# willi-menapace/PlayableEnvironments

Hardware: AMD Instinct MI355X
Metric: Mrays/s (higher is better)
Workload: dtype f32; 1 GPU; tennis renderer, 256x256 frame per GPU (rank r renders the frame of seed 1234 + r), 4 objects, 64+128 hierarchical samples/ray (coarse+fine networks), eval - BASELINE.json configs[1]; rays_per_gpu=65536, frames_per_gpu=1, parallelism=frame shard x1

## Files before the change

playableenvironments_amd/csrc/mlp.hip:

```cpp
#include "pr_common.h"
#include "mlp_tile.h"

#include <cstddef>

#include <stdarg.h>
#include <stdlib.h>

namespace pr {


int compute_dims(const pr_object_model_t& m, ModelDims* d) {
    PR_REQUIRE(m.kind == 0 || m.kind == 1, "unknown nerf model kind %d", m.kind);
    PR_REQUIRE(m.octaves >= 0 && m.octaves <= PR_MAX_OCTAVES, "octaves %d out of range", m.octaves);
    d->din = m.kind == 0 ? 3 : 6;
    d->enc = d->din + 2 * d->din * m.octaves;
    d->enc_pad = round_up(d->enc, 32);
    d->W = m.layers_width;
    d->Wpad = round_up(d->W, 32);
    d->W2 = m.layers_width / 2;
    d->W2pad = round_up(d->W2, 32);
    d->F = m.output_features;
    d->Fpad = round_up(d->F, 32);
    PR_REQUIRE(d->enc_pad <= MAX_ENC, "encoding width %d exceeds %d", d->enc, MAX_ENC);
    PR_REQUIRE(d->W >= 2 && d->Wpad <= MAX_WIDTH, "layers_width %d unsupported (max %d)", d->W, MAX_WIDTH);
// ... 397 lines not shown
        if (first) {
            row[ch] = g;
            row[p.Wpad + ch] = b;
        } else {
            row[2 * p.Wpad + ch] = g;
            row[2 * p.Wpad + p.W2pad + ch] = b;
        }
    }
}

__global__ __launch_bounds__(256) void k_adain_fold(FoldParams p) { adain_fold_body(p); }

struct FoldGroup { FoldParams job[PR_MAX_OBJECTS]; };
__global__ __launch_bounds__(256) void k_adain_fold_group(FoldGroup g) {
    const FoldParams& p = g.job[blockIdx.z];
    if ((int)blockIdx.x >= p.frames || (int)blockIdx.y * 256 >= p.Wpad + p.W2pad) return;
    adain_fold_body(p);
}

int launch_adain_fold(const FoldParams& p, hipStream_t s) {
    PR_REQUIRE(p.affine1.weight && p.affine1.bias && p.affine4.weight && p.affine4.bias && p.bn1_mean && p.bn1_var &&
                   p.bn4_mean && p.bn4_var,
               "AdaIN parameters missing");
    PR_REQUIRE(p.affine1.out_features == 2 * p.W && p.affine1.in_features == p.S, "features_head.1 affine shape");
    PR_REQUIRE(p.affine4.out_features == 2 * p.W2 && p.affine4.in_features == p.S, "features_head.4 affine shape");
    hipLaunchKernelGGL(k_adain_fold, dim3(p.frames, (p.Wpad + p.W2pad + 255) / 256), dim3(256), 0, s, p);
    PR_LAUNCH_CHECK();
    return PR_OK;
}

int launch_adain_fold_group(const FoldParams* jobs, int count, hipStream_t s) {
    PR_REQUIRE(count >= 1 && count <= PR_MAX_OBJECTS, "adain fold group: %d objects", count);
    static thread_local FoldGroup g;
    int frames = 0, blocks = 0;
    for (int k = 0; k < count; ++k) {
        const FoldParams& p = jobs[k];
        PR_REQUIRE(p.affine1.weight && p.affine1.bias && p.affine4.weight && p.affine4.bias && p.bn1_mean && p.bn1_var &&
                       p.bn4_mean && p.bn4_var,
                   "AdaIN parameters missing");
        PR_REQUIRE(p.affine1.out_features == 2 * p.W && p.affine1.in_features == p.S, "features_head.1 affine shape");
        PR_REQUIRE(p.affine4.out_features == 2 * p.W2 && p.affine4.in_features == p.S, "features_head.4 affine shape");
        g.job[k] = p;
        frames = std::max(frames, p.frames);
        blocks = std::max(blocks, (p.Wpad + p.W2pad + 255) / 256);
    }
    hipLaunchKernelGGL(k_adain_fold_group, dim3(frames, blocks, count), dim3(256), 0, s, g);
    PR_LAUNCH_CHECK();
    return PR_OK;
}


__device__ __forceinline__ void head_on_tile(Smem& S, const MlpParams& p, EncRegs& enc, int valid_rows) {
    for (int l = p.n_backbone; l < p.n_layers; ++l) run_layer(p.layers[l], S, p, 0, 0, enc);
    write_rows_indirect(S, p.feat, p.F, p.F, p.ones_col);
    if (threadIdx.x == 0 && p.head_count) atomicAdd(p.head_count, valid_rows);
    __syncthreads();
}

__device__ __forceinline__ int gated_head(Smem& S, const MlpParams& p, int tile_base, int pending, EncRegs& enc) {
    const int tid = threadIdx.x, lane = tid & 63;
    const unsigned long long live = __ballot((S.flags[lane] & 4) != 0);
    const int L = __popcll(live);
    float* pact = p.pend_act + (size_t)blockIdx.x * TILE_M * p.Wpad;
    int* pmeta = p.pend_meta + (size_t)blockIdx.x * TILE_M * 2;
    const unsigned long long below = (1ull << lane) - 1ull;
    const int w4 = p.Wpad >> 2;
    if (L == 0) {
        __syncthreads();
        return pending;
    }
    if (pending + L >= TILE_M) {
        const int need = TILE_M - L;
        if (tid == 0) S.uniform_frame = 1;
        if (tid < TILE_M) {
            if ((live >> tid) & 1ull) {
                S.dest[tid] = tile_base + tid;
                S.src[tid] = -1;
            } else {
                const int slot = pending - need + __popcll(~live & below);
                S.src[tid] = slot;
                S.dest[tid] = pmeta[2 * slot];
                S.frame[tid] = pmeta[2 * slot + 1];
            }
        }
        __syncthreads();
        if (need) {
            for (int idx = tid; idx < TILE_M * w4; idx += MLP_THREADS) {
                const int row = idx / w4, c = (idx - row * w4) * 4;
                const int slot = S.src[row];
                if (slot >= 0)
                    *reinterpret_cast<float4*>(S.X + row * LDX + c) = *reinterpret_cast<const float4*>(pact + (size_t)slot * p.Wpad + c);
            }
        }
        if (tid < TILE_M && S.frame[tid] != S.frame[0]) S.uniform_frame = 0;
        __syncthreads();
        head_on_tile(S, p, enc, TILE_M);
        return pending - need;
    }
    if (tid < TILE_M) {
        int slot = -1;
        if ((live >> tid) & 1ull) {
            slot = pending + __popcll(live & below);
            pmeta[2 * slot] = tile_base + tid;
            pmeta[2 * slot + 1] = S.frame[tid];
        }
        S.src[tid] = slot;
    }
    __syncthreads();
    for (int idx = tid; idx < TILE_M * w4; idx += MLP_THREADS) {
        const int row = idx / w4, c = (idx - row * w4) * 4;
        const int slot = S.src[row];
        if (slot >= 0)
            *reinterpret_cast<float4*>(pact + (size_t)slot * p.Wpad + c) = *reinterpret_cast<const float4*>(S.X + row * LDX + c);
    }
    __syncthreads();
    return pending + L;
}

__device__ __forceinline__ void gated_head_flush(Smem& S, const MlpParams& p, int pending, EncRegs& enc) {
    if (pending <= 0) return;
    const int tid = threadIdx.x;
    const float* pact = p.pend_act + (size_t)blockIdx.x * TILE_M * p.Wpad;
    const int* pmeta = p.pend_meta + (size_t)blockIdx.x * TILE_M * 2;
    const int w4 = p.Wpad >> 2;
    if (tid == 0) S.uniform_frame = 1;
    if (tid < TILE_M) {
        const bool has = tid < pending;
        S.dest[tid] = has ? pmeta[2 * tid] : -1;
        S.frame[tid] = pmeta[2 * (has ? tid : 0) + 1];
    }
    __syncthreads();
    for (int idx = tid; idx < pending * w4; idx += MLP_THREADS) {
        const int row = idx / w4, c = (idx - row * w4) * 4;
        *reinterpret_cast<float4*>(S.X + row * LDX + c) = *reinterpret_cast<const float4*>(pact + (size_t)row * p.Wpad + c);
    }
    if (tid < TILE_M && S.frame[tid] != S.frame[0]) S.uniform_frame = 0;
    __syncthreads();
    head_on_tile(S, p, enc, pending);
}


__device__ __forceinline__ void count_stat_rows(const Smem& S, const MlpParams& p) {
    if (p.phase == 1 && threadIdx.x < 64) {
        const int alive = __popcll(__ballot((S.flags[threadIdx.x] & 3) == 3));
        if (threadIdx.x == 0 && alive) atomicAdd(p.stat_count, alive);
    }
}

__device__ __forceinline__ void flush_column_stats(const ColumnStats& cs, const MlpParams& p, int nblk) {
    const int wave = threadIdx.x >> 6, lane = threadIdx.x & 63;
    if (lane >= 32) return;
#pragma unroll
    for (int blk = 0; blk < 2; ++blk) {
        const int cb = wave + blk * MLP_WAVES;
        if (cb >= nblk) continue;
        const int col = cb * 32 + lane;
        const double s1 = blk ? cs.s1[1] : cs.s1[0], s2 = blk ? cs.s2[1] : cs.s2[0];
        if (s1 != 0.0 || s2 != 0.0) {
            atomicAdd(p.stats + col, s1);
            atomicAdd(p.stats + p.h_out_width + col, s2);
        }
    }
}

#ifdef PR_MLP_TRACE
__device__ unsigned long long g_mlp_trace[1024][12];
#define PR_TRACE_MARK(i) if (threadIdx.x == 0) g_mlp_trace[blockIdx.x][i] = wall_clock64()
#else
#define PR_TRACE_MARK(i)
#endif

template <bool TRAIN, bool GROUP, bool SPLIT = false, bool SIGMA_ONLY = false>
__device__ __forceinline__ void mlp_tile_loop(const MlpParams& p) {
    extern __shared__ __attribute__((aligned(16))) char smem_raw[];
    Smem& S = *reinterpret_cast<Smem*>(smem_raw);
    const int tid = threadIdx.x;
    const int total = *p.total;
    PR_PHASE_BEGIN();
    if (GROUP) {
        __syncthreads();
        if (tid == 0) S.next_tile = atomicAdd(p.tile_counter, 1);
    }
    for (int i = tid; i <= p.Wpad; i += MLP_THREADS) S.head_w[i] = p.sigma_w[i];
    __syncthreads();
    int pending = 0;
    EncRegs enc;
    ColumnStats cstats;
    cstats.s1[0] = cstats.s1[1] = cstats.s2[0] = cstats.s2[1] = 0.0;
    const bool dynamic_tiles = GROUP || (!TRAIN && p.tile_counter != nullptr);
    for (int tile = GROUP ? S.next_tile : (int)blockIdx.x; tile * TILE_M < total; tile = S.next_tile) {
        const int tile_base = tile * TILE_M;
        PR_PHASE_T0();
#ifdef PR_MLP_TRACE
        if (GROUP && !TRAIN && tid == 0) g_mlp_trace[blockIdx.x][5 + (p.positions == 4 ? 0 : 1)] += 1;
#endif
        int claimed = 0;
        if (tid == 0) S.uniform_frame = 1;
        if (SPLIT && tid == 0) S.tile_max[0] = S.tile_max[1] = 0;
        if (tid < TILE_M) {
            const int idx = tile_base + tid;
            const bool valid = idx < total;
            const int src = valid ? idx : tile_base;
            const int flat = p.rec_flat[src];
            const int frame = flat / p.samples_per_frame;
            S.flat[tid] = flat;
            S.frame[tid] = frame;
            S.flags[tid] = valid ? 3 : 0;
            if (p.kind == 0) {
                S.pos[tid * 8 + 0] = p.rec_pos[(size_t)src * 3 + 0];
                S.pos[tid * 8 + 1] = p.rec_pos[(size_t)src * 3 + 1];
                S.pos[tid * 8 + 2] = p.rec_pos[(size_t)src * 3 + 2];
            } else {
                const int ray = (flat - frame * p.samples_per_frame) / p.positions;
                const ObjRay rr = object_ray(p.w2o + (size_t)frame * p.w2o_stride, p.ray_origins + (size_t)frame * 3,
                                             p.ray_directions + ((size_t)frame * p.rays + ray) * 3);
                const float nrm = sqrtf(__fadd_rn(__fadd_rn(__fmul_rn(rr.d[0], rr.d[0]), __fmul_rn(rr.d[1], rr.d[1])),
                                                  __fmul_rn(rr.d[2], rr.d[2])));
                for (int a = 0; a < 3; ++a) {
                    S.pos[tid * 8 + a] = __fdiv_rn(rr.o[a], p.size[a]);
                    S.pos[tid * 8 + 3 + a] = __fdiv_rn(rr.d[a], nrm);
                }
            }
        }
        __syncthreads();
        if (tid < TILE_M && S.frame[tid] != S.frame[0]) S.uniform_frame = 0;
        PR_PHASE(0);

        int cur = p.has_bender ? 0 : 1;
        if (p.has_bender) {
            fill_bender_input(S, p, enc, false, SPLIT ? &S.tile_max[0] : nullptr);
            __syncthreads();
            if (TRAIN && p.save_bin) write_tile_rows(S, p.save_bin, p.bin_pad, p.bin_pad, tile_base, false);
            for (int l = 0; l < p.b_count; ++l) {
                if (TRAIN) {
                    run_layer<false, true, false, SPLIT>(p.b_layers[l], S, p, tile_base, 1, enc, nullptr,
                                           p.save_bbits ? reinterpret_cast<unsigned long long*>(p.save_bbits + (size_t)l * p.save_bbits_stride) +
                                                              (size_t)tile * p.BWpad : nullptr, nullptr, &cur);
                } else {
                    run_layer(p.b_layers[l], S, p, tile_base, 1, enc);
                }
                if (TRAIN && p.save_bact) write_tile_rows(S, p.save_bact + (size_t)l * p.save_bact_stride, p.BWpad, p.BWpad, tile_base, false);
            }
            if (SPLIT && tid == 0) S.tile_max[cur ^ 1] = 0;
            for (int s = tid >> 3; s < TILE_M; s += MLP_THREADS / 8) {
                float out[3];
                row_dots(S, s, as_global(p.b_out), p.BWpad, p.BWpad, 3, out);
                if ((tid & 7) != 0) continue;
                float d[3], bent[3];
                if (TRAIN && p.save_braw && (S.flags[s] & 1))
                    for (int a = 0; a < 3; ++a) p.save_braw[(size_t)(tile_base + s) * 3 + a] = out[a];
                for (int a = 0; a < 3; ++a) {
                    const float x = S.pos[s * 8 + a];
                    float dl = __fmul_rn(out[a], p.size[a]);
                    dl = nan_max(dl, __fsub_rn(p.lo[a], x));
                    dl = nan_min(dl, __fsub_rn(p.hi[a], x));
                    if (p.canonical) dl = __fmul_rn(dl, 0.0f);
                    d[a] = dl;
                    bent[a] = __fadd_rn(x, dl);
                    S.pos[s * 8 + a] = bent[a];
                }
                if (S.flags[s] & 1) {
                    if (p.dispmag)
                        p.dispmag[S.flat[s]] = sqrtf(__fadd_rn(__fadd_rn(__fmul_rn(d[0], d[0]), __fmul_rn(d[1], d[1])),
                                                               __fmul_rn(d[2], d[2])));
                    if (TRAIN && p.save_delta)
                        for (int a = 0; a < 3; ++a) p.save_delta[(size_t)(tile_base + s) * 3 + a] = d[a];
                    if (p.delta_dense)
                        for (int a = 0; a < 3; ++a) p.delta_dense[(size_t)S.flat[s] * 3 + a] = d[a];
                    if (!in_box(bent[0], bent[1], bent[2], p.lo, p.hi)) S.flags[s] &= ~2;
                }
            }
            __syncthreads();
        }

        PR_PHASE(1);
        fill_nerf_input(S, p, enc, false, SPLIT ? &S.tile_max[cur ^ 1] : nullptr);
        cur ^= 1;
        __syncthreads();
        PR_PHASE(2);
        if (TRAIN && p.save_enc) write_tile_rows(S, p.save_enc, p.enc_pad, p.enc_pad, tile_base, false);

        for (int l = 0; l < p.n_backbone; ++l) {
            if (TRAIN) {
                run_layer<false, true, false, SPLIT>(p.layers[l], S, p, tile_base, 0, enc, nullptr,
                                       p.save_bits
                                           ? reinterpret_cast<unsigned long long*>(p.save_bits + (size_t)l * p.save_bits_stride) + (size_t)tile * p.Wpad
                                           : nullptr, nullptr, &cur);
            } else {
                run_layer(p.layers[l], S, p, tile_base, 0, enc);
            }
            PR_PHASE(10);
            if (TRAIN && p.save_act)
                write_tile_rows(S, p.save_act + (size_t)l * p.save_act_stride, p.Wpad, p.Wpad, tile_base, false);
            PR_PHASE(11);
        }

        PR_PHASE(15);
        if (dynamic_tiles && tid == 0) claimed = atomicAdd(p.tile_counter, 1);
        if (p.kind == 0) {
            for (int s = tid >> 3; s < TILE_M; s += MLP_THREADS / 8) {
                float sg;
                row_dots(S, s, S.head_w, p.Wpad, p.Wpad, 1, &sg);
                if ((tid & 7) == 0 && (S.flags[s] & 3) == 3) {
                    const float sv = p.in_scene[(size_t)S.frame[s] * p.in_scene_stride] ? sg + S.head_w[p.Wpad] : p.empty_alpha;
                    p.sigma[S.flat[s]] = sv;
                    if (!(sv <= 0.f)) S.flags[s] |= 4;
                }
            }
        } else if (tid < TILE_M) {
            if (S.flags[tid] & 1) {
                const bool present = p.in_scene[(size_t)S.frame[tid] * p.in_scene_stride] != 0;
                p.sigma[S.flat[tid]] = present ? 10.0f : p.empty_alpha;
                if (present || !(p.empty_alpha <= 0.f)) S.flags[tid] |= 4;
            }
        }

        if (tid == 0) S.next_tile = GROUP ? claimed : (dynamic_tiles ? (int)gridDim.x + claimed : tile + (int)gridDim.x);
        PR_PHASE(7);
        if (SIGMA_ONLY) {
            __syncthreads();
        } else if (!TRAIN && p.gate) {
            __syncthreads();
            if (!(p.empty_alpha <= 0.f)) {
                for (int idx = tid; idx < TILE_M * p.F; idx += MLP_THREADS) {
                    const int row = idx / p.F;
                    if ((S.flags[row] & 3) == 1) p.feat[(size_t)(tile_base + row) * p.F + (idx - row * p.F)] = 0.f;
                }
            }
            pending = gated_head(S, p, tile_base, pending, enc);
            PR_PHASE(8);
        } else if (!TRAIN) {
            for (int l = p.n_backbone; l < p.n_layers; ++l) run_layer(p.layers[l], S, p, tile_base, 0, enc);
            PR_PHASE(15);
            write_tile_rows(S, p.feat, p.F, p.F, tile_base, true, p.ones_col);
            __syncthreads();
            PR_PHASE(8);
        } else {
            Layer raw = p.layers[p.n_backbone];
            raw.epi = EPI_FEATURES;
            run_layer<false, false, true, SPLIT>(raw, S, p, tile_base, 0, enc, nullptr, nullptr, &cstats, &cur);
            PR_PHASE(12);
            if (tid < TILE_M && (S.flags[tid] & 1)) p.row_flags[tile_base + tid] = S.flags[tid];
            write_tile_rows(S, p.h_out, p.h_out_width, p.h_out_width, tile_base, false);
            count_stat_rows(S, p);
            PR_PHASE(13);
            __syncthreads();
            PR_PHASE(14);
        }
    }
    if (!TRAIN && !SIGMA_ONLY && p.gate) gated_head_flush(S, p, pending, enc);
    if (TRAIN) flush_column_stats(cstats, p, p.layers[p.n_backbone].nblk);
    PR_PHASE_FLUSH();
}

__global__ __launch_bounds__(MLP_THREADS, MLP_BLOCKS_PER_CU) void k_mlp_mfma(MlpParams p) { mlp_tile_loop<false, false>(p); }
__global__ __launch_bounds__(MLP_THREADS, MLP_BLOCKS_PER_CU) void k_mlp_mfma_train(MlpParams p) { mlp_tile_loop<true, false>(p); }
__global__ __launch_bounds__(MLP_THREADS, MLP_BLOCKS_PER_CU) void k_mlp_sigma(MlpParams p) { mlp_tile_loop<false, false, false, true>(p); }
__global__ __launch_bounds__(MLP_THREADS, MLP_BLOCKS_PER_CU) void k_mlp_mfma_group(MlpParams j0, MlpParams j1, MlpParams j2, MlpParams j3,
                                                                                   int count) {
    PR_TRACE_MARK(0);
    mlp_tile_loop<false, true>(j0);
    PR_TRACE_MARK(1);
    if (count > 1) mlp_tile_loop<false, true>(j1);
    PR_TRACE_MARK(2);
    if (count > 2) mlp_tile_loop<false, true>(j2);
    PR_TRACE_MARK(3);
    if (count > 3) mlp_tile_loop<false, true>(j3);
    PR_TRACE_MARK(4);
}

__global__ __launch_bounds__(MLP_THREADS, MLP_BLOCKS_PER_CU) void k_mlp_sigma_group(MlpParams j0, MlpParams j1, MlpParams j2, MlpParams j3,
                                                                                    int count) {
    mlp_tile_loop<false, true, false, true>(j0);
    if (count > 1) mlp_tile_loop<false, true, false, true>(j1);
    if (count > 2) mlp_tile_loop<false, true, false, true>(j2);
    if (count > 3) mlp_tile_loop<false, true, false, true>(j3);
}

#ifdef PR_MLP_TRACE
extern "C" int pr_debug_mlp_trace(unsigned long long* out) {
    (void)hipDeviceSynchronize();
    return hipMemcpyFromSymbol(out, HIP_SYMBOL(g_mlp_trace), sizeof(unsigned long long) * 1024 * 12) == hipSuccess ? 0 : 1;
}
#endif

__global__ __launch_bounds__(MLP_THREADS, MLP_BLOCKS_PER_CU) void k_mlp_mfma_train_group(MlpParams j0, MlpParams j1, MlpParams j2, MlpParams j3,
                                                                                         int count) {
    mlp_tile_loop<true, true>(j0);
    if (count > 1) mlp_tile_loop<true, true>(j1);
// ... 627 lines not shown
    PR_LAUNCH_CHECK();
    return PR_OK;
}

int launch_chain_bwd(const ChainBwdParams& c, int max_rows, hipStream_t s) {
    if (max_rows <= 0) return PR_OK;
    int cu_count = 0;
    PR_TRY(prepare_kernel(reinterpret_cast<const void*>(k_chain_bwd), (int)sizeof(Smem), &cu_count));
    const int max_tiles = (max_rows + TILE_M - 1) / TILE_M;
    const int resident = cu_count * MLP_BLOCKS_PER_CU;
    ProfileScope scope(2, s);
    hipLaunchKernelGGL(k_chain_bwd, dim3(max_tiles < resident ? max_tiles : resident), dim3(MLP_THREADS), sizeof(Smem), s, c);
    PR_LAUNCH_CHECK();
    return PR_OK;
}

__global__ __launch_bounds__(512) void k_probe_mfma(int iterations, float* sink, int random_operands) {
    f32x16 acc0, acc1;
#pragma unroll
    for (int i = 0; i < 16; ++i) {
        acc0[i] = 0.f;
        acc1[i] = 1.f;
    }
    float a = 1.0f + threadIdx.x * 1e-6f, b = 1.0f - threadIdx.x * 1e-6f;
    unsigned int x = 0x9E3779B9u * (threadIdx.x + 1) + blockIdx.x;
    for (int it = 0; it < iterations; ++it) {
        if (random_operands) {
            x ^= x << 13; x ^= x >> 17; x ^= x << 5;
            a = __uint_as_float((x & 0x807FFFFFu) | 0x3F000000u);
            b = __uint_as_float(((x * 2654435761u) & 0x807FFFFFu) | 0x3F000000u);
        }
        acc0 = __builtin_amdgcn_mfma_f32_32x32x2f32(a, b, acc0, 0, 0, 0);
        acc1 = __builtin_amdgcn_mfma_f32_32x32x2f32(b, a, acc1, 0, 0, 0);
        acc0 = __builtin_amdgcn_mfma_f32_32x32x2f32(a, a, acc0, 0, 0, 0);
        acc1 = __builtin_amdgcn_mfma_f32_32x32x2f32(b, b, acc1, 0, 0, 0);
        acc0 = __builtin_amdgcn_mfma_f32_32x32x2f32(a, b, acc0, 0, 0, 0);
        acc1 = __builtin_amdgcn_mfma_f32_32x32x2f32(b, a, acc1, 0, 0, 0);
        acc0 = __builtin_amdgcn_mfma_f32_32x32x2f32(a, a, acc0, 0, 0, 0);
        acc1 = __builtin_amdgcn_mfma_f32_32x32x2f32(b, b, acc1, 0, 0, 0);
        if (random_operands && (it & 63) == 63) {
#pragma unroll
            for (int i = 0; i < 16; ++i) {
                acc0[i] *= 0.001f;
                acc1[i] *= 0.001f;
            }
        }
    }
    float s = 0.f;
#pragma unroll
    for (int i = 0; i < 16; ++i) s += acc0[i] + acc1[i];
    if (s == 123.456f) sink[0] = s;
}

}

extern "C" int pr_probe_mfma_f32(int32_t iterations, int32_t random_operands, double* tflops, double* milliseconds, void* stream) {
    PR_REQUIRE(iterations > 0 && tflops, "pr_probe_mfma_f32: bad argument");
    int dev = 0;
    PR_CHECK_HIP(hipGetDevice(&dev));
    hipDeviceProp_t prop;
    PR_CHECK_HIP(hipGetDeviceProperties(&prop, dev));
    const int cus = prop.multiProcessorCount;
    float* sink = nullptr;
    PR_CHECK_HIP(hipMalloc(&sink, sizeof(float)));
    hipEvent_t e0, e1;
    PR_CHECK_HIP(hipEventCreate(&e0));
    PR_CHECK_HIP(hipEventCreate(&e1));
    hipStream_t s = (hipStream_t)stream;
    constexpr int PROBE_WAVES = 8;
    hipLaunchKernelGGL(pr::k_probe_mfma, dim3(cus), dim3(64 * PROBE_WAVES), 0, s, 16, sink, random_operands);
    PR_CHECK_HIP(hipEventRecord(e0, s));
    hipLaunchKernelGGL(pr::k_probe_mfma, dim3(cus), dim3(64 * PROBE_WAVES), 0, s, iterations, sink, random_operands);
    PR_CHECK_HIP(hipEventRecord(e1, s));
    PR_CHECK_HIP(hipEventSynchronize(e1));
    float ms = 0.f;
    PR_CHECK_HIP(hipEventElapsedTime(&ms, e0, e1));
    const double flop = (double)cus * PROBE_WAVES * (double)iterations * 8.0 * (2.0 * 32 * 32 * 2);
    *tflops = flop / (ms * 1e-3) / 1e12;
    if (milliseconds) *milliseconds = ms;
    PR_CHECK_HIP(hipEventDestroy(e0));
    PR_CHECK_HIP(hipEventDestroy(e1));
    PR_CHECK_HIP(hipFree(sink));
    return PR_OK;
}

namespace pr {
}

extern "C" int pr_packed_size(const pr_object_model_t* model, size_t* bytes) {
    PR_REQUIRE(model && bytes, "pr_packed_size: NULL argument");
    pr::ModelDims d;
    pr::PackedLayout l;
    PR_TRY(pr::compute_dims(*model, &d));
    PR_TRY(pr::compute_layout(*model, d, &l));
    *bytes = (size_t)l.total * sizeof(float);
    return PR_OK;
}

extern "C" int pr_pack_model(const pr_object_model_t* model, int32_t precision, void* packed, size_t packed_bytes, void* stream) {
    PR_REQUIRE(precision == PR_PRECISION_FP32 || precision == PR_PRECISION_F16X3 || precision == PR_PRECISION_F16,
               "pr_pack_model: precision must be one of PR_PRECISION_*");
    PR_REQUIRE(model && packed, "pr_pack_model: NULL argument");
    PR_REQUIRE(((uintptr_t)packed & 15) == 0, "pr_pack_model: packed buffer must be 16-byte aligned");
    pr::ModelDims d;
    pr::PackedLayout l;
    PR_TRY(pr::compute_dims(*model, &d));
    PR_TRY(pr::compute_layout(*model, d, &l));
    PR_REQUIRE(packed_bytes >= (size_t)l.total * sizeof(float), "pr_pack_model: buffer too small (%zu < %zu)",
               packed_bytes, (size_t)l.total * sizeof(float));
    pr::PackJobs jobs;
    jobs.seg_kind = precision ? 2 : 0;
    PR_TRY(pr::build_pack_jobs(*model, d, l, static_cast<float*>(packed), &jobs));
    hipLaunchKernelGGL(pr::k_pack, dim3(64, jobs.n), dim3(256), 0, (hipStream_t)stream, jobs);
    PR_LAUNCH_CHECK();
    return PR_OK;
}

extern "C" int pr_pack_models(int32_t count, const pr_object_model_t* const* models, const int32_t* precisions, void* const* packed,
                              const size_t* packed_bytes, void* stream) {
    PR_REQUIRE(count >= 0 && (count == 0 || (models && precisions && packed && packed_bytes)), "pr_pack_models: NULL argument");
    static thread_local pr::PackJobs all, one;
    all.n = 0;
    all.seg_kind = 0;
    auto flush = [&]() -> int {
        if (all.n == 0) return PR_OK;
        hipLaunchKernelGGL(pr::k_pack, dim3(64, all.n), dim3(256), 0, (hipStream_t)stream, all);
        PR_LAUNCH_CHECK();
        all.n = 0;
        return PR_OK;
    };
// ... 19 lines not shown
```

playableenvironments_amd/csrc/mlp_tile.h:

```cpp
#pragma once
#include "pr_common.h"

#include <cstddef>

namespace pr {

typedef float f32x16 __attribute__((ext_vector_type(16)));

constexpr int HEAD_SIGMA = MAX_WIDTH + 8;
constexpr int HEAD_BENDER = 0;
struct Smem {
    int uniform_frame;
    int next_tile;
    int tile_max[2];
    float head_w[HEAD_SIGMA + HEAD_BENDER];
    float X[TILE_M * LDX];
    float pos[TILE_M * 8];
    int flat[TILE_M];
    int frame[TILE_M];
    int flags[TILE_M];
    int dest[TILE_M];
    int src[TILE_M];
#ifdef PR_MLP_TIMING
    unsigned long long phase_acc[16];
#endif
};
static_assert(sizeof(Smem) * MLP_BLOCKS_PER_CU <= 160 * 1024 - MLP_BLOCKS_PER_CU * 1024, "the workgroups of one CU must fit its LDS");
static_assert(offsetof(Smem, head_w) % 16 == 0 && offsetof(Smem, X) % 16 == 0 && offsetof(Smem, pos) % 16 == 0,
              "16-byte LDS reads of the activation tile");


__device__ __forceinline__ int acc_row(int reg, int half) { return (reg & 3) + 8 * (reg >> 2) + 4 * half; }

__device__ __forceinline__ float pe_element(const float* v, int din, int enc, int j, const float* octave_weights) {
    if (j < din) return v[j];
    if (j >= enc) return 0.f;
    const int jj = j - din;
    const int k = jj / (2 * din);
    const int rem = jj - k * 2 * din;
    const int fn = rem / din;
    const int ax = rem - fn * din;
    const float arg = __fmul_rn(ldexpf(1.0f, k), v[ax]);
    float e = fn ? cosf(arg) : sinf(arg);
    if (octave_weights) e = __fmul_rn(e, octave_weights[k]);
    return e;
}

#define PR_ACC_ROW(i) (((i) & 3) + 8 * ((i) >> 2))

__device__ __forceinline__ void store_relu(const f32x16& acc, float* base) {
#pragma unroll
    for (int i = 0; i < 16; ++i) base[PR_ACC_ROW(i) * LDX] = acc[i] > 0.f ? acc[i] : 0.f;
}

__device__ __forceinline__ void store_adain_uniform(const f32x16& acc, float* base, float g, float b) {
#pragma unroll
    for (int i = 0; i < 16; ++i) {
        const float v = fmaf(acc[i], g, b);
        base[PR_ACC_ROW(i) * LDX] = v > 0.f ? v : 0.f;
    }
}

__device__ __forceinline__ void store_adain_rows(const f32x16& acc, Smem& S, const MlpParams& p, int row0, int col,
                                             int goff, int boff) {
#pragma unroll
    for (int c = 0; c < 4; ++c) {
        float g[4], b[4];
#pragma unroll
        for (int i = 0; i < 4; ++i) {
            const float* tab = p.adain + (size_t)S.frame[row0 + PR_ACC_ROW(4 * c + i)] * p.adain_stride;
            g[i] = tab[goff];
            b[i] = tab[boff];
        }
#pragma unroll
        for (int i = 0; i < 4; ++i) {
// ... 331 lines not shown
            obh = wpB[at]; obl = wpB[at + 64];
            __builtin_amdgcn_sched_barrier(0);
            PR_STEP_MFMAS_H(e0, e1, eah, eal, ebh, ebl);
            o0 = split_fragment_scaled_h(xl, xh, scale); o1 = split_fragment_scaled_h(yl, yh, scale);
            if (drain) drain_next(*drain, X, cursor);
            __builtin_amdgcn_sched_barrier(0);
        }
        {
            const int sn = (s + 2 < ks) ? s + 2 : s;
            const float* an = ap + 16 * sn;
            xl = *reinterpret_cast<const float4*>(an); xh = *reinterpret_cast<const float4*>(an + 4);
            yl = *reinterpret_cast<const float4*>(an + 32 * LDX); yh = *reinterpret_cast<const float4*>(an + 32 * LDX + 4);
            const size_t at = (size_t)sn * 128;
            eah = wpA[at]; eal = wpA[at + 64];
            ebh = wpB[at]; ebl = wpB[at + 64];
            __builtin_amdgcn_sched_barrier(0);
            PR_STEP_MFMAS_H(o0, o1, oah, oal, obh, obl);
            e0 = split_fragment_scaled_h(xl, xh, scale); e1 = split_fragment_scaled_h(yl, yh, scale);
            if (drain) drain_next(*drain, X, cursor);
            __builtin_amdgcn_sched_barrier(0);
        }
    }
    __builtin_amdgcn_s_setprio(0);
}

template <bool BWD, bool BITS, bool STATS, bool SPLIT>
__device__ __forceinline__ void run_layer(const Layer& L, Smem& S, const MlpParams& p, int tile_base, int input_kind, EncRegs& enc,
                                          const BwdEpilogue* bwd, unsigned long long* bits_out, ColumnStats* stats, int* cur_slot) {
    const int wave = threadIdx.x >> 6, lane = threadIdx.x & 63;
    const int r = lane & 31, half = lane >> 5;
    const int nblk = L.nblk;
    int slot = SPLIT ? *cur_slot : 0;
    int k = SPLIT ? tile_scale_log2(S.tile_max[slot]) : 0;
    const int cbA = wave, cbB = wave + MLP_WAVES;
    const bool active = cbA < nblk;
    const bool two = cbB < nblk;
    PR_PHASE_T0();
    f32x16 a00, a01, a10, a11;
    {
        float biasA = (L.bias != nullptr && active) ? as_global(L.bias)[cbA * 32 + r] : 0.f;
        float biasB = (L.bias != nullptr && two) ? as_global(L.bias)[cbB * 32 + r] : 0.f;
        if (SPLIT) {
            biasA = ldexpf(biasA, k + TRAIN_SPLIT_WEIGHT_SCALE_LOG2);
            biasB = ldexpf(biasB, k + TRAIN_SPLIT_WEIGHT_SCALE_LOG2);
        }
#pragma unroll
        for (int i = 0; i < 16; ++i) {
            a00[i] = biasA;
            a01[i] = biasA;
            a10[i] = biasB;
            a11[i] = biasB;
        }
    }
    for (int sidx = 0; sidx < L.nseg; ++sidx) {
        const Seg& sg = L.seg[sidx];
        if (!BWD && sg.src == 1 && sidx > 0) {
            __syncthreads();
            int* refill_slot = SPLIT ? &S.tile_max[slot ^ 1] : nullptr;
            if (input_kind == 1) fill_bender_input(S, p, enc, true, refill_slot); else fill_nerf_input(S, p, enc, true, refill_slot);
            __syncthreads();
            if (SPLIT) {
                slot ^= 1;
                const int k1 = tile_scale_log2(S.tile_max[slot]);
                const float shift = ldexpf(1.0f, k1 - k);
#pragma unroll
                for (int i = 0; i < 16; ++i) {
                    a00[i] *= shift;
                    a01[i] *= shift;
                    a10[i] *= shift;
                    a11[i] *= shift;
                }
                k = k1;
            }
        }
        if (SPLIT && threadIdx.x == 0) S.tile_max[slot ^ 1] = 0;
        if (!active) continue;
        if (SPLIT) {
            PR_PHASE_COUNT(8, 1000000ull * (sg.kq >> 1));
            PR_PHASE_COUNT(9, 1000000ull);
            tile_products_f16x3_lean(sg, nblk, S.X, a00, a01, a10, a11, ldexpf(1.0f, k));
            continue;
        }
        PR_PHASE_COUNT(8, 1000000ull * (sg.kq >> 1));
        PR_PHASE_COUNT(9, 1000000ull);
        __builtin_amdgcn_s_setprio(1);
        const int kq = sg.kq;
        const float* ap = S.X + r * LDX + half * 4 * kq;
        const auto* wpA = as_global(reinterpret_cast<const f32x4_t*>(sg.w)) + (size_t)cbA * kq * 64 + lane;
        float4 x0e = *reinterpret_cast<const float4*>(ap);
        float4 x1e = *reinterpret_cast<const float4*>(ap + 32 * LDX);
        float4 x0o = *reinterpret_cast<const float4*>(ap + 4);
        float4 x1o = *reinterpret_cast<const float4*>(ap + 32 * LDX + 4);
        if (two) {
            const auto* wpB = as_global(reinterpret_cast<const f32x4_t*>(sg.w)) + (size_t)cbB * kq * 64 + lane;
            f32x4_t wAe = wpA[0], wBe = wpB[0];
            __builtin_amdgcn_sched_barrier(0);
            f32x4_t wAo = wpA[64], wBo = wpB[64];
            __builtin_amdgcn_sched_barrier(0);
            for (int q = 0; q < kq; q += 2) {
                const int qe = (q + 2 < kq) ? q + 2 : q, qo = (q + 3 < kq) ? q + 3 : q + 1;
                PR_MFMA4(a00, x0e, wAe);
                PR_MFMA4(a01, x1e, wAe);
                PR_MFMA4(a10, x0e, wBe);
                PR_MFMA4(a11, x1e, wBe);
                wAe = wpA[(size_t)qe * 64];
                wBe = wpB[(size_t)qe * 64];
// ... 90 lines not shown
        if (active) {
            const unsigned char* bits = reinterpret_cast<const unsigned char*>(S.pos);
            const int bpr = bwd->mask_bytes_per_row;
            for (int blk = 0; blk < (two ? 2 : 1); ++blk) {
                const int col = (blk ? cbB : cbA) * 32 + r;
                const f32x16& lo = blk ? a10 : a00;
                const f32x16& hi = blk ? a11 : a01;
                float* x0 = S.X + (4 * half) * LDX + col;
                const unsigned char* b0 = bits + (4 * half) * bpr + (col >> 3);
                const int bit = col & 7;
#pragma unroll
                for (int i = 0; i < 16; ++i) {
                    const int ro = PR_ACC_ROW(i);
                    x0[ro * LDX] = ((b0[ro * bpr] >> bit) & 1) ? lo[i] : 0.f;
                    x0[(ro + 32) * LDX] = ((b0[(ro + 32) * bpr] >> bit) & 1) ? hi[i] : 0.f;
                }
            }
        }
        __syncthreads();
        return;
    }
    __syncthreads();
    PR_PHASE(4);
    if (active) {
        for (int blk = 0; blk < (two ? 2 : 1); ++blk) {
            const int col = (blk ? cbB : cbA) * 32 + r;
            const f32x16& lo = blk ? a10 : a00;
            const f32x16& hi = blk ? a11 : a01;
            float* x0 = S.X + (4 * half) * LDX + col;
            if (L.epi == EPI_RELU) {
                store_relu(lo, x0);
                store_relu(hi, x0 + 32 * LDX);
                if (SPLIT) {
                    float biggest = 0.f;
#pragma unroll
                    for (int i = 0; i < 16; ++i) biggest = fmaxf(biggest, fmaxf(lo[i], hi[i]));
                    commit_tile_max(fmaxf(biggest, 0.f), &S.tile_max[slot ^ 1]);
                }
                if (BITS && bits_out) {
                    unsigned int mlo = 0u, mhi = 0u;
#pragma unroll
                    for (int i = 0; i < 16; ++i) {
                        mlo |= (lo[i] > 0.f ? 1u : 0u) << PR_ACC_ROW(i);
                        mhi |= (hi[i] > 0.f ? 1u : 0u) << PR_ACC_ROW(i);
                    }
                    mlo <<= 4 * half;
                    mhi <<= 4 * half;
                    mlo |= (unsigned int)__shfl_xor((int)mlo, 32, 64);
                    mhi |= (unsigned int)__shfl_xor((int)mhi, 32, 64);
                    if (half == 0) bits_out[col] = ((unsigned long long)mhi << 32) | mlo;
                }
            } else if (L.epi == EPI_ADAIN_RELU) {
                const int bofs = L.nblk * 32;
                if (S.uniform_frame) {
                    const float* tab = p.adain + (size_t)S.frame[0] * p.adain_stride + L.adain_off;
                    const float g = tab[col], b = tab[bofs + col];
                    store_adain_uniform(lo, x0, g, b);
                    store_adain_uniform(hi, x0 + 32 * LDX, g, b);
                } else {
                    store_adain_rows(lo, S, p, 4 * half, col, L.adain_off + col, L.adain_off + bofs + col);
                    store_adain_rows(hi, S, p, 4 * half + 32, col, L.adain_off + col, L.adain_off + bofs + col);
                }
            } else {
                store_plain(lo, x0);
                store_plain(hi, x0 + 32 * LDX);
                if (STATS && stats) {
                    const unsigned long long mine = __ballot((S.flags[lane] & 3) == 3) >> (4 * half);
                    const unsigned int mlo = (unsigned int)mine, mhi = (unsigned int)(mine >> 32);
                    double s1 = 0.0, s2 = 0.0;
#pragma unroll
                    for (int i = 0; i < 16; ++i) {
                        const double x0 = ((mlo >> PR_ACC_ROW(i)) & 1u) ? (double)lo[i] : 0.0;
                        s1 += x0;
                        s2 = fma(x0, x0, s2);
                        const double x1 = ((mhi >> PR_ACC_ROW(i)) & 1u) ? (double)hi[i] : 0.0;
                        s1 += x1;
                        s2 = fma(x1, x1, s2);
                    }
                    s1 += __shfl_xor(s1, 32, 64);
                    s2 += __shfl_xor(s2, 32, 64);
                    if (blk == 0) {
                        stats->s1[0] += s1;
                        stats->s2[0] += s2;
                    } else {
                        stats->s1[1] += s1;
                        stats->s2[1] += s2;
                    }
                }
            }
        }
    }
    PR_PHASE(5);
    __syncthreads();
    PR_PHASE(6);
}

template <class W>
__device__ __forceinline__ void row_dots(const Smem& S, int s, W w, int width, int wstride, int nout, float* out) {
    const int part = threadIdx.x & 7;
    float acc[3] = {0.f, 0.f, 0.f};
    for (int k = part; k < width; k += 8) {
        const float x = S.X[s * LDX + k];
        for (int a = 0; a < nout; ++a) acc[a] = fmaf(x, w[a * wstride + k], acc[a]);
    }
    for (int a = 0; a < nout; ++a) {
        float v = acc[a];
        v += __shfl_xor(v, 1, 64);
        v += __shfl_xor(v, 2, 64);
        v += __shfl_xor(v, 4, 64);
        out[a] = v;
    }
}

template <class V>
__device__ __forceinline__ V homogeneous_chunk(V v, int c, int ones_col) {
    if (c + 3 >= ones_col) {
        v.x = c < ones_col ? v.x : (c == ones_col ? 1.0f : 0.f);
        v.y = c + 1 < ones_col ? v.y : (c + 1 == ones_col ? 1.0f : 0.f);
        v.z = c + 2 < ones_col ? v.z : (c + 2 == ones_col ? 1.0f : 0.f);
        v.w = c + 3 < ones_col ? v.w : (c + 3 == ones_col ? 1.0f : 0.f);
    }
    return v;
}

__device__ __forceinline__ void write_tile_rows(const Smem& S, float* dst, int width, int stride, int tile_base, bool zero_dead,
                                                int ones_col = 0) {
    const int tid = threadIdx.x;
    const float* src = S.X;
    const int ld = LDX;
    if ((width & 3) == 0 && (stride & 3) == 0) {
        const int w4 = width >> 2;
        const int count = TILE_M * w4;
        constexpr int BATCH = 4;
        const bool aligned = (MLP_THREADS % w4) == 0;
        const int rstep = MLP_THREADS / w4;
        typedef float f32x4_nt __attribute__((ext_vector_type(4)));
        for (int base = tid; base < count; base += MLP_THREADS * BATCH) {
            int row[BATCH], c[BATCH], fl[BATCH];
            const int row0 = base / w4, c0 = (base - row0 * w4) * 4;
#pragma unroll
            for (int q = 0; q < BATCH; ++q) {
                const int idx = base + q * MLP_THREADS;
                if (aligned) {
                    row[q] = row0 + q * rstep;
                    c[q] = c0;
                } else {
                    row[q] = idx / w4;
                    c[q] = (idx - row[q] * w4) * 4;
                }
                if (idx >= count) row[q] = 0, c[q] = 0;
                fl[q] = idx < count ? S.flags[row[q]] : 0;
            }
            f32x4_nt v[BATCH];
#pragma unroll
            for (int q = 0; q < BATCH; ++q) v[q] = *reinterpret_cast<const f32x4_nt*>(src + row[q] * ld + c[q]);
#pragma unroll
            for (int q = 0; q < BATCH; ++q) {
                if (fl[q] & 1) {
                    if (ones_col) v[q] = homogeneous_chunk(v[q], c[q], ones_col);
                    if (zero_dead && !(fl[q] & 2)) v[q] = f32x4_nt{0.f, 0.f, 0.f, 0.f};
                    __builtin_nontemporal_store(v[q], reinterpret_cast<f32x4_nt*>(dst + (size_t)(tile_base + row[q]) * stride + c[q]));
                }
            }
        }
    } else {
        for (int idx = tid; idx < TILE_M * width; idx += MLP_THREADS) {
            const int row = idx / width, c = idx - row * width;
            const int fl = S.flags[row];
            if (fl & 1) dst[(size_t)(tile_base + row) * stride + c] = (zero_dead && !(fl & 2)) ? 0.f : src[row * ld + c];
        }
    }
}

__device__ __forceinline__ void write_rows_indirect(const Smem& S, float* dst, int width, int stride, int ones_col = 0) {
    const int tid = threadIdx.x;
    if ((width & 3) == 0 && (stride & 3) == 0) {
        const int w4 = width >> 2;
        for (int idx = tid; idx < TILE_M * w4; idx += MLP_THREADS) {
            const int row = idx / w4, c = (idx - row * w4) * 4;
            const int d = S.dest[row];
            if (d >= 0) {
                const float4 v = *reinterpret_cast<const float4*>(S.X + row * LDX + c);
                typedef float f32x4_nt __attribute__((ext_vector_type(4)));
                f32x4_nt nt = {v.x, v.y, v.z, v.w};
                if (ones_col) nt = homogeneous_chunk(nt, c, ones_col);
                __builtin_nontemporal_store(nt, reinterpret_cast<f32x4_nt*>(dst + (size_t)d * stride + c));
            }
        }
    } else {
        for (int idx = tid; idx < TILE_M * width; idx += MLP_THREADS) {
            const int row = idx / width, c = idx - row * width;
            const int d = S.dest[row];
            if (d >= 0) dst[(size_t)d * stride + c] = S.X[row * LDX + c];
        }
    }
}

__device__ __forceinline__ void build_relu_mask_bits(unsigned char* bits, const float* acts, int ld, int width_pad, int tile_base,
                                                     int rows_valid) {
    const int c8n = width_pad >> 3;
    for (int idx = threadIdx.x; idx < TILE_M * c8n; idx += MLP_THREADS) {
        const int row = idx / c8n, c8 = idx - row * c8n;
        unsigned int byte = 0;
        if (row < rows_valid) {
            const float* src = acts + (size_t)(tile_base + row) * ld + 8 * c8;
            const float4 a = *reinterpret_cast<const float4*>(src);
            const float4 b = *reinterpret_cast<const float4*>(src + 4);
            byte = (a.x > 0.f ? 1u : 0u) | (a.y > 0.f ? 2u : 0u) | (a.z > 0.f ? 4u : 0u) | (a.w > 0.f ? 8u : 0u) |
                   (b.x > 0.f ? 16u : 0u) | (b.y > 0.f ? 32u : 0u) | (b.z > 0.f ? 64u : 0u) | (b.w > 0.f ? 128u : 0u);
        }
        bits[idx] = (unsigned char)byte;
    }
}

}
```

Measured before the change: 0.3300 Mrays/s.

## Prefetch next tile records, batch pending-row exchange, hoist AdaIN table loads

The tile loop now loads the next tile's flat index and positions into registers before the head stage runs, so the global load latency is hidden behind later work. The gated-head pending-row copies are rewritten as batched 4-wide loads and stores driven by a running row/column cursor and ballot masks. This drops the shared src array and one barrier. write_rows_indirect gets the same batching, and the per-frame AdaIN gain and shift values are loaded once before the segment loop rather than in the epilogue. The change also adds phase-timing markers and a new MFMA probe kernel, and it costs some extra registers for the prefetched records.

```diff
diff --git a/playableenvironments_amd/csrc/mlp.hip b/playableenvironments_amd/csrc/mlp.hip
--- a/playableenvironments_amd/csrc/mlp.hip
+++ b/playableenvironments_amd/csrc/mlp.hip
@@ -473,9 +473,47 @@
 
 __device__ __forceinline__ void head_on_tile(Smem& S, const MlpParams& p, EncRegs& enc, int valid_rows) {
     for (int l = p.n_backbone; l < p.n_layers; ++l) run_layer(p.layers[l], S, p, 0, 0, enc);
+    PR_PHASE_T0();
     write_rows_indirect(S, p.feat, p.F, p.F, p.ones_col);
     if (threadIdx.x == 0 && p.head_count) atomicAdd(p.head_count, valid_rows);
     __syncthreads();
+    PR_PHASE(12);
+}
+
+template <bool POP>
+__device__ __forceinline__ void exchange_pending_rows(Smem& S, float* pact, int Wpad, unsigned long long rows, int first) {
+    const int w4 = Wpad >> 2;
+    const int count = TILE_M * w4;
+    constexpr int BATCH = 4;
+    ChunkCursor k = chunk_begin(w4);
+    for (int base = threadIdx.x; base < count; base += MLP_THREADS * BATCH) {
+        int row[BATCH], c[BATCH], slot[BATCH];
+#pragma unroll
+        for (int q = 0; q < BATCH; ++q) {
+            const bool inside = base + q * MLP_THREADS < count;
+            row[q] = inside ? k.row : 0;
+            c[q] = inside ? 4 * k.c4 : 0;
+            const bool takes_part = inside && ((rows >> row[q]) & 1ull);
+            slot[q] = takes_part ? first + __popcll(rows & ((1ull << row[q]) - 1ull)) : -1;
+            chunk_next(k, w4);
+        }
+        f32x4_t v[BATCH];
+#pragma unroll
+        for (int q = 0; q < BATCH; ++q) {
+            if (POP) {
+                if (slot[q] >= 0) v[q] = *(as_global(reinterpret_cast<const f32x4_t*>(pact + (size_t)slot[q] * Wpad + c[q])));
+            } else {
+                v[q] = *reinterpret_cast<const f32x4_t*>(S.X + row[q] * LDX + c[q]);
+            }
+        }
+#pragma unroll
+        for (int q = 0; q < BATCH; ++q) {
+            if (slot[q] >= 0) {
+                if (POP) *reinterpret_cast<f32x4_t*>(S.X + row[q] * LDX + c[q]) = v[q];
+                else *(as_global(reinterpret_cast<f32x4_t*>(pact + (size_t)slot[q] * Wpad + c[q]))) = v[q];
+            }
+        }
+    }
 }
 
 __device__ __forceinline__ int gated_head(Smem& S, const MlpParams& p, int tile_base, int pending, EncRegs& enc) {
@@ -485,9 +523,10 @@
     float* pact = p.pend_act + (size_t)blockIdx.x * TILE_M * p.Wpad;
     int* pmeta = p.pend_meta + (size_t)blockIdx.x * TILE_M * 2;
     const unsigned long long below = (1ull << lane) - 1ull;
-    const int w4 = p.Wpad >> 2;
+    PR_PHASE_T0();
     if (L == 0) {
         __syncthreads();
+        PR_PHASE(13);
         return pending;
     }
     if (pending + L >= TILE_M) {
@@ -496,45 +535,28 @@
         if (tid < TILE_M) {
             if ((live >> tid) & 1ull) {
                 S.dest[tid] = tile_base + tid;
-                S.src[tid] = -1;
             } else {
                 const int slot = pending - need + __popcll(~live & below);
-                S.src[tid] = slot;
                 S.dest[tid] = pmeta[2 * slot];
                 S.frame[tid] = pmeta[2 * slot + 1];
             }
         }
+        if (need) exchange_pending_rows<true>(S, pact, p.Wpad, ~live, pending - need);
         __syncthreads();
-        if (need) {
-            for (int idx = tid; idx < TILE_M * w4; idx += MLP_THREADS) {
-                const int row = idx / w4, c = (idx - row * w4) * 4;
-                const int slot = S.src[row];
-                if (slot >= 0)
-                    *reinterpret_cast<float4*>(S.X + row * LDX + c) = *reinterpret_cast<const float4*>(pact + (size_t)slot * p.Wpad + c);
-            }
-        }
         if (tid < TILE_M && S.frame[tid] != S.frame[0]) S.uniform_frame = 0;
         __syncthreads();
+        PR_PHASE(13);
         head_on_tile(S, p, enc, TILE_M);
         return pending - need;
     }
-    if (tid < TILE_M) {
-        int slot = -1;
-        if ((live >> tid) & 1ull) {
-            slot = pending + __popcll(live & below);
-            pmeta[2 * slot] = tile_base + tid;
-            pmeta[2 * slot + 1] = S.frame[tid];
-        }
-        S.src[tid] = slot;
-    }
+    if (tid < TILE_M && ((live >> tid) & 1ull)) {
+        const int slot = pending + __popcll(live & below);
+        pmeta[2 * slot] = tile_base + tid;
+        pmeta[2 * slot + 1] = S.frame[tid];
+    }
+    exchange_pending_rows<false>(S, pact, p.Wpad, live, pending);
     __syncthreads();
-    for (int idx = tid; idx < TILE_M * w4; idx += MLP_THREADS) {
-        const int row = idx / w4, c = (idx - row * w4) * 4;
-        const int slot = S.src[row];
-        if (slot >= 0)
-            *reinterpret_cast<float4*>(pact + (size_t)slot * p.Wpad + c) = *reinterpret_cast<const float4*>(S.X + row * LDX + c);
-    }
-    __syncthreads();
+    PR_PHASE(13);
     return pending + L;
 }
 
@@ -591,6 +613,21 @@
 #define PR_TRACE_MARK(i)
 #endif
 
+struct TileRecords { int flat; float pos[3]; };
+static_assert(TILE_M == 64, "the rows of a tile are loaded by the lanes of wave 0");
+__device__ __forceinline__ TileRecords request_tile_records(const MlpParams& p, int tile_base, int total) {
+    const int idx = tile_base + (int)threadIdx.x;
+    const int src = idx < total ? idx : tile_base;
+    TileRecords r = {as_global(p.rec_flat)[src], {0.f, 0.f, 0.f}};
+    if (p.kind == 0) {
+        const auto* pos = as_global(p.rec_pos) + (size_t)src * 3;
+        r.pos[0] = pos[0];
+        r.pos[1] = pos[1];
+        r.pos[2] = pos[2];
+    }
+    return r;
+}
+
 template <bool TRAIN, bool GROUP, bool SPLIT = false, bool SIGMA_ONLY = false>
 __device__ __forceinline__ void mlp_tile_loop(const MlpParams& p) {
     extern __shared__ __attribute__((aligned(16))) char smem_raw[];
@@ -609,7 +646,10 @@
     ColumnStats cstats;
     cstats.s1[0] = cstats.s1[1] = cstats.s2[0] = cstats.s2[1] = 0.0;
     const bool dynamic_tiles = GROUP || (!TRAIN && p.tile_counter != nullptr);
-    for (int tile = GROUP ? S.next_tile : (int)blockIdx.x; tile * TILE_M < total; tile = S.next_tile) {
+    const int first_tile = GROUP ? S.next_tile : (int)blockIdx.x;
+    TileRecords rec = {0, {0.f, 0.f, 0.f}};
+    if (tid < TILE_M && first_tile * TILE_M < total) rec = request_tile_records(p, first_tile * TILE_M, total);
+    for (int tile = first_tile; tile * TILE_M < total; tile = S.next_tile) {
         const int tile_base = tile * TILE_M;
         PR_PHASE_T0();
 #ifdef PR_MLP_TRACE
@@ -619,18 +659,16 @@
         if (tid == 0) S.uniform_frame = 1;
         if (SPLIT && tid == 0) S.tile_max[0] = S.tile_max[1] = 0;
         if (tid < TILE_M) {
-            const int idx = tile_base + tid;
-            const bool valid = idx < total;
-            const int src = valid ? idx : tile_base;
-            const int flat = p.rec_flat[src];
+            const bool valid = tile_base + tid < total;
+            const int flat = rec.flat;
             const int frame = flat / p.samples_per_frame;
             S.flat[tid] = flat;
             S.frame[tid] = frame;
             S.flags[tid] = valid ? 3 : 0;
             if (p.kind == 0) {
-                S.pos[tid * 8 + 0] = p.rec_pos[(size_t)src * 3 + 0];
-                S.pos[tid * 8 + 1] = p.rec_pos[(size_t)src * 3 + 1];
-                S.pos[tid * 8 + 2] = p.rec_pos[(size_t)src * 3 + 2];
+                S.pos[tid * 8 + 0] = rec.pos[0];
+                S.pos[tid * 8 + 1] = rec.pos[1];
+                S.pos[tid * 8 + 2] = rec.pos[2];
             } else {
                 const int ray = (flat - frame * p.samples_per_frame) / p.positions;
                 const ObjRay rr = object_ray(p.w2o + (size_t)frame * p.w2o_stride, p.ray_origins + (size_t)frame * 3,
@@ -736,7 +774,12 @@
             }
         }
 
-        if (tid == 0) S.next_tile = GROUP ? claimed : (dynamic_tiles ? (int)gridDim.x + claimed : tile + (int)gridDim.x);
+        const int next = GROUP ? claimed : (dynamic_tiles ? (int)gridDim.x + claimed : tile + (int)gridDim.x);
+        if (tid == 0) S.next_tile = next;
+        if (tid < TILE_M) {
+            const int next_base = __builtin_amdgcn_readfirstlane(next) * TILE_M;
+            if (next_base < total) rec = request_tile_records(p, next_base, total);
+        }
         PR_PHASE(7);
         if (SIGMA_ONLY) {
             __syncthreads();
@@ -749,13 +792,13 @@
                 }
             }
             pending = gated_head(S, p, tile_base, pending, enc);
-            PR_PHASE(8);
+            PR_PHASE(14);
         } else if (!TRAIN) {
             for (int l = p.n_backbone; l < p.n_layers; ++l) run_layer(p.layers[l], S, p, tile_base, 0, enc);
             PR_PHASE(15);
             write_tile_rows(S, p.feat, p.F, p.F, tile_base, true, p.ones_col);
             __syncthreads();
-            PR_PHASE(8);
+            PR_PHASE(14);
         } else {
             Layer raw = p.layers[p.n_backbone];
             raw.epi = EPI_FEATURES;
@@ -1489,6 +1532,66 @@
     if (s == 123.456f) sink[0] = s;
 }
 
+template <bool SHARED>
+__global__ __launch_bounds__(512) void k_probe_mfma_step(int iterations, float* sink) {
+    f32x16 a00, a01, a10, a11;
+#pragma unroll
+    for (int i = 0; i < 16; ++i) {
+        a00[i] = 0.f;
+        a01[i] = 1.f;
+        a10[i] = 0.f;
+        a11[i] = 1.f;
+    }
+    unsigned int x = 0x9E3779B9u * (threadIdx.x + 1) + blockIdx.x;
+#define PR_PROBE_MFMA(acc, a, b)                                  \
+    acc = __builtin_amdgcn_mfma_f32_32x32x2f32(a, b, acc, 0, 0, 0); \
+    __builtin_amdgcn_sched_barrier(0)
+    for (int it = 0; it < iterations; ++it) {
+        x ^= x << 13; x ^= x >> 17; x ^= x << 5;
+        float x0[4], x1[4], wA[4], wB[4];
+#pragma unroll
+        for (int j = 0; j < 4; ++j) {
+            x0[j] = __uint_as_float(((x * (2654435761u + 8u * j)) & 0x807FFFFFu) | 0x3F000000u);
+            x1[j] = __uint_as_float(((x * (2246822519u + 8u * j)) & 0x807FFFFFu) | 0x3F000000u);
+            wA[j] = __uint_as_float(((x * (3266489917u + 8u * j)) & 0x807FFFFFu) | 0x3F000000u);
+            wB[j] = __uint_as_float(((x * (668265263u + 8u * j)) & 0x807FFFFFu) | 0x3F000000u);
+        }
+        __builtin_amdgcn_sched_barrier(0);
+        if (SHARED) {
+#pragma unroll
+            for (int j = 0; j < 4; ++j) {
+                PR_PROBE_MFMA(a00, x0[j], wA[j]);
+                PR_PROBE_MFMA(a01, x1[j], wA[j]);
+                PR_PROBE_MFMA(a10, x0[j], wB[j]);
+                PR_PROBE_MFMA(a11, x1[j], wB[j]);
+            }
+        } else {
+#pragma unroll
+            for (int j = 0; j < 4; ++j) { PR_PROBE_MFMA(a00, x0[j], wA[j]); }
+#pragma unroll
+            for (int j = 0; j < 4; ++j) { PR_PROBE_MFMA(a01, x1[j], wA[j]); }
+#pragma unroll
+            for (int j = 0; j < 4; ++j) { PR_PROBE_MFMA(a10, x0[j], wB[j]); }
+#pragma unroll
+            for (int j = 0; j < 4; ++j) { PR_PROBE_MFMA(a11, x1[j], wB[j]); }
+        }
+        if ((it & 31) == 31) {
+#pragma unroll
+            for (int i = 0; i < 16; ++i) {
+                a00[i] *= 0.001f;
+                a01[i] *= 0.001f;
+                a10[i] *= 0.001f;
+                a11[i] *= 0.001f;
+            }
+        }
+    }
+#undef PR_PROBE_MFMA
+    float s = 0.f;
+#pragma unroll
+    for (int i = 0; i < 16; ++i) s += a00[i] + a01[i] + a10[i] + a11[i];
+    if (s == 123.456f) sink[0] = s;
+}
+
 }
 
 extern "C" int pr_probe_mfma_f32(int32_t iterations, int32_t random_operands, double* tflops, double* milliseconds, void* stream) {
@@ -1505,14 +1608,20 @@
     PR_CHECK_HIP(hipEventCreate(&e1));
     hipStream_t s = (hipStream_t)stream;
     constexpr int PROBE_WAVES = 8;
-    hipLaunchKernelGGL(pr::k_probe_mfma, dim3(cus), dim3(64 * PROBE_WAVES), 0, s, 16, sink, random_operands);
+    const bool step = random_operands == 2 || random_operands == 3;
+    const auto launch = [&](int n) {
+        if (random_operands == 2) hipLaunchKernelGGL(pr::k_probe_mfma_step<false>, dim3(cus), dim3(64 * PROBE_WAVES), 0, s, n, sink);
+        else if (random_operands == 3) hipLaunchKernelGGL(pr::k_probe_mfma_step<true>, dim3(cus), dim3(64 * PROBE_WAVES), 0, s, n, sink);
+        else hipLaunchKernelGGL(pr::k_probe_mfma, dim3(cus), dim3(64 * PROBE_WAVES), 0, s, n, sink, random_operands);
+    };
+    launch(16);
     PR_CHECK_HIP(hipEventRecord(e0, s));
-    hipLaunchKernelGGL(pr::k_probe_mfma, dim3(cus), dim3(64 * PROBE_WAVES), 0, s, iterations, sink, random_operands);
+    launch(iterations);
     PR_CHECK_HIP(hipEventRecord(e1, s));
     PR_CHECK_HIP(hipEventSynchronize(e1));
     float ms = 0.f;
     PR_CHECK_HIP(hipEventElapsedTime(&ms, e0, e1));
-    const double flop = (double)cus * PROBE_WAVES * (double)iterations * 8.0 * (2.0 * 32 * 32 * 2);
+    const double flop = (double)cus * PROBE_WAVES * (double)iterations * (step ? 16.0 : 8.0) * (2.0 * 32 * 32 * 2);
     *tflops = flop / (ms * 1e-3) / 1e12;
     if (milliseconds) *milliseconds = ms;
     PR_CHECK_HIP(hipEventDestroy(e0));
diff --git a/playableenvironments_amd/csrc/mlp_tile.h b/playableenvironments_amd/csrc/mlp_tile.h
--- a/playableenvironments_amd/csrc/mlp_tile.h
+++ b/playableenvironments_amd/csrc/mlp_tile.h
@@ -20,7 +20,6 @@
     int frame[TILE_M];
     int flags[TILE_M];
     int dest[TILE_M];
-    int src[TILE_M];
 #ifdef PR_MLP_TIMING
     unsigned long long phase_acc[16];
 #endif
@@ -458,6 +457,18 @@
             a11[i] = biasB;
         }
     }
+    const bool adain_uniform = !BWD && L.epi == EPI_ADAIN_RELU && S.uniform_frame != 0;
+    float gainA = 0.f, shiftA = 0.f, gainB = 0.f, shiftB = 0.f;
+    if (adain_uniform && active) {
+        const auto* tab = as_global(p.adain) + (size_t)S.frame[0] * p.adain_stride + L.adain_off;
+        const int bofs = nblk * 32;
+        gainA = tab[cbA * 32 + r];
+        shiftA = tab[bofs + cbA * 32 + r];
+        if (two) {
+            gainB = tab[cbB * 32 + r];
+            shiftB = tab[bofs + cbB * 32 + r];
+        }
+    }
     for (int sidx = 0; sidx < L.nseg; ++sidx) {
         const Seg& sg = L.seg[sidx];
         if (!BWD && sg.src == 1 && sidx > 0) {
@@ -654,9 +665,8 @@
                 }
             } else if (L.epi == EPI_ADAIN_RELU) {
                 const int bofs = L.nblk * 32;
-                if (S.uniform_frame) {
-                    const float* tab = p.adain + (size_t)S.frame[0] * p.adain_stride + L.adain_off;
-                    const float g = tab[col], b = tab[bofs + col];
+                if (adain_uniform) {
+                    const float g = blk ? gainB : gainA, b = blk ? shiftB : shiftA;
                     store_adain_uniform(lo, x0, g, b);
                     store_adain_uniform(hi, x0 + 32 * LDX, g, b);
                 } else {
@@ -725,6 +735,23 @@
     return v;
 }
 
+struct ChunkCursor { int row, c4, drow, dc4; };
+__device__ __forceinline__ ChunkCursor chunk_begin(int w4) {
+    ChunkCursor k;
+    k.row = (int)threadIdx.x / w4;
+    k.c4 = (int)threadIdx.x - k.row * w4;
+    k.drow = MLP_THREADS / w4;
+    k.dc4 = MLP_THREADS - k.drow * w4;
+    return k;
+}
+__device__ __forceinline__ void chunk_next(ChunkCursor& k, int w4) {
+    k.c4 += k.dc4;
+    k.row += k.drow;
+    const int wrap = k.c4 >= w4 ? 1 : 0;
+    k.c4 -= wrap ? w4 : 0;
+    k.row += wrap;
+}
+
 __device__ __forceinline__ void write_tile_rows(const Smem& S, float* dst, int width, int stride, int tile_base, bool zero_dead,
                                                 int ones_col = 0) {
     const int tid = threadIdx.x;
@@ -734,24 +761,17 @@
         const int w4 = width >> 2;
         const int count = TILE_M * w4;
         constexpr int BATCH = 4;
-        const bool aligned = (MLP_THREADS % w4) == 0;
-        const int rstep = MLP_THREADS / w4;
         typedef float f32x4_nt __attribute__((ext_vector_type(4)));
+        ChunkCursor k = chunk_begin(w4);
         for (int base = tid; base < count; base += MLP_THREADS * BATCH) {
             int row[BATCH], c[BATCH], fl[BATCH];
-            const int row0 = base / w4, c0 = (base - row0 * w4) * 4;
 #pragma unroll
             for (int q = 0; q < BATCH; ++q) {
                 const int idx = base + q * MLP_THREADS;
-                if (aligned) {
-                    row[q] = row0 + q * rstep;
-                    c[q] = c0;
-                } else {
-                    row[q] = idx / w4;
-                    c[q] = (idx - row[q] * w4) * 4;
-                }
-                if (idx >= count) row[q] = 0, c[q] = 0;
+                row[q] = idx < count ? k.row : 0;
+                c[q] = idx < count ? 4 * k.c4 : 0;
                 fl[q] = idx < count ? S.flags[row[q]] : 0;
+                chunk_next(k, w4);
             }
             f32x4_nt v[BATCH];
 #pragma unroll
@@ -778,15 +798,29 @@
     const int tid = threadIdx.x;
     if ((width & 3) == 0 && (stride & 3) == 0) {
         const int w4 = width >> 2;
-        for (int idx = tid; idx < TILE_M * w4; idx += MLP_THREADS) {
-            const int row = idx / w4, c = (idx - row * w4) * 4;
-            const int d = S.dest[row];
-            if (d >= 0) {
-                const float4 v = *reinterpret_cast<const float4*>(S.X + row * LDX + c);
-                typedef float f32x4_nt __attribute__((ext_vector_type(4)));
-                f32x4_nt nt = {v.x, v.y, v.z, v.w};
-                if (ones_col) nt = homogeneous_chunk(nt, c, ones_col);
-                __builtin_nontemporal_store(nt, reinterpret_cast<f32x4_nt*>(dst + (size_t)d * stride + c));
+        const int count = TILE_M * w4;
+        constexpr int BATCH = 4;
+        typedef float f32x4_nt __attribute__((ext_vector_type(4)));
+        ChunkCursor k = chunk_begin(w4);
+        for (int base = tid; base < count; base += MLP_THREADS * BATCH) {
+            int row[BATCH], c[BATCH], d[BATCH];
+#pragma unroll
+            for (int q = 0; q < BATCH; ++q) {
+                const int idx = base + q * MLP_THREADS;
+                row[q] = idx < count ? k.row : 0;
+                c[q] = idx < count ? 4 * k.c4 : 0;
+                d[q] = idx < count ? S.dest[row[q]] : -1;
+                chunk_next(k, w4);
+            }
+            f32x4_nt v[BATCH];
+#pragma unroll
+            for (int q = 0; q < BATCH; ++q) v[q] = *reinterpret_cast<const f32x4_nt*>(S.X + row[q] * LDX + c[q]);
+#pragma unroll
+            for (int q = 0; q < BATCH; ++q) {
+                if (d[q] >= 0) {
+                    if (ones_col) v[q] = homogeneous_chunk(v[q], c[q], ones_col);
+                    __builtin_nontemporal_store(v[q], reinterpret_cast<f32x4_nt*>(dst + (size_t)d[q] * stride + c[q]));
+                }
             }
         }
     } else {
```

After: 0.3274 Mrays/s. No clear change (-0.8%).
